# sanweiliti/RoHM

Hardware: AMD Instinct MI355X
Metric: denoised 145-frame clips/sec @1000 DDPM steps (higher is better)
Workload: dtype f32

## Files before the change

rohm_amd/csrc/encoder_chain.hip:

```cpp
#include <type_traits>
#include "common.h"
#include "gemm_sched.h"
#include "attention_tile.h"

namespace rohm {

typedef float f32x16c __attribute__((ext_vector_type(16)));

namespace chain {

constexpr int BM = 144, BK = kGemmBK, NRB = BM / 16;
constexpr int A_UNITS = BM * 8, A_ITERS = (A_UNITS + 255) / 256;
constexpr int kMaxBN = 384;
constexpr int kZone = 2 * (BM + kMaxBN) * BK;
constexpr int kLdsFloats = kZone + 512 + 4 * BM * 2;
constexpr int kSc1 = 16;

struct PhaseArgs {
    const float* A; int lda;
    const float* W; int ldw;
    float* C; int ldc;
    int K;
    const float* bias;
    const float* R; int ldr;
    const float* gamma; const float* beta; float eps; int ln_dim;
    int qcols; float qscale;
    int S; const float* tab; const float* tab0; int ldtab, ldtab0, tab_by_row;
    int m0, n0;
    float* row_stats; unsigned tag28; int tn, tiles_n;
    unsigned* err; unsigned xcc1; int fault;
};

__device__ __forceinline__ int head_row(int n0, int t) { return ((t % 96) >> 5) * 512 + n0 + (t / 96) * 32 + (t & 31); }

template <int BN, bool HEAD = false>
__device__ __forceinline__ void prefetch_w(const float* W, int ldw, int n0, float* smem, int tid, int wave_u) {
    constexpr int B_ITERS = BN * 8 / 256;
    float* Bs = smem + 2 * BM * BK;
#pragma unroll
    for (int buf = 0; buf < 2; ++buf)
#pragma unroll
        for (int i = 0; i < B_ITERS; ++i) {
            const int u = tid + i * 256;
            const int row = u >> 3;
            const int slot = (u & 7) ^ ((row >> 1) & 7);
            const float* src = W + (size_t)(HEAD ? head_row(n0, row) : n0 + row) * ldw + slot * 4 + buf * BK;
            __builtin_amdgcn_global_load_lds((const __attribute__((address_space(1))) void*)src,
                                             (__attribute__((address_space(3))) void*)(Bs + buf * (BN * BK) + (i * 256 + wave_u) * 4), 16, 0, 0);
        }
}

__device__ __forceinline__ void group_sync(unsigned long long* flags, int tn, int G, unsigned tag, unsigned xcc1, unsigned* err, int tid) {
    asm volatile("s_waitcnt vmcnt(0)" ::: "memory");
    __syncthreads();
    if (tid == 0) {
        flags[tn] = ((unsigned long long)xcc1 << 32) | tag;
        asm volatile("" ::: "memory");
    }
    if (tid < G && tid != tn) {
        for (int it = 0;; ++it) {
            const unsigned long long f = __hip_atomic_load(flags + tid, __ATOMIC_RELAXED, __HIP_MEMORY_SCOPE_AGENT);
            if ((unsigned)f == tag && (f >> 32) != 0ull) {
                if ((unsigned)(f >> 32) != xcc1) __hip_atomic_store(err, 2u, __ATOMIC_RELAXED, __HIP_MEMORY_SCOPE_AGENT);
                break;
            }
            __builtin_amdgcn_s_sleep(1);
            if ((it & 127) == 127 && __hip_atomic_load(err, __ATOMIC_RELAXED, __HIP_MEMORY_SCOPE_AGENT) != 0u) break;
            if (it > (1 << 19)) {
                __hip_atomic_store(err, 1u, __ATOMIC_RELAXED, __HIP_MEMORY_SCOPE_AGENT);
                break;
            }
        }
    }
    __syncthreads();
}

template <int BN, int EPI, bool PREF, bool SC1, bool REFETCH, bool HEAD = false, typename AfterLoop>
__device__ __forceinline__ void gemm_phase(const PhaseArgs& p, float* smem, const int tid, AfterLoop&& after_loop,
                                           AtQFrags<2>* q_out = nullptr) {
    static_assert(EPI == EPI_BIAS_RES_LN || EPI == EPI_BIAS_GELU || EPI == EPI_QKV || EPI == EPI_EMBED, "chain phases: LN tail, GELU, QKV, embed");
    static_assert(!HEAD || (EPI == EPI_QKV && BN == 3 * AT_DH), "the head-aligned tile is one head's q | k | v");
    constexpr int WN = BN / 4;
    constexpr int NCB = WN / 16;
    constexpr int B_ITERS = BN * 8 / 256;
    constexpr int PIECES = A_ITERS + B_ITERS;
    constexpr int AUX = SC1 ? kSc1 : 0;

    float* As = smem;
    float* Bs = smem + 2 * BM * BK;
    float* lds_dummy = smem + kZone;
    float* const zone = lds_dummy + 512;
    float* const colrow = HEAD ? smem + 2 * AT_TILE : zone;
    static_assert(!HEAD || 2 * AT_TILE + 512 <= AT_LDS_FLOATS, "head-aligned tile: the bias row overruns the stack's LDS");

    const int lane = tid & 63;
    const int wave = tid >> 6;
    const int li = lane & 15, lg = lane >> 4;
    const int wave_u = __builtin_amdgcn_readfirstlane(wave) * 64;
    const int m0 = p.m0, n0 = p.n0;

    const float* a_src[A_ITERS];
#pragma unroll
    for (int i = 0; i < A_ITERS; ++i) {
        const int u = tid + i * 256;
        const int row = (u < A_UNITS) ? (u >> 3) : 0;
        const int slot = (u & 7) ^ ((row >> 1) & 7);
        a_src[i] = p.A + (size_t)(m0 + row) * p.lda + slot * 4;
    }
    const float* b_src[B_ITERS];
#pragma unroll
    for (int i = 0; i < B_ITERS; ++i) {
        const int u = tid + i * 256;
        const int row = u >> 3;
        const int slot = (u & 7) ^ ((row >> 1) & 7);
        b_src[i] = p.W + (size_t)(HEAD ? head_row(n0, row) : n0 + row) * p.ldw + slot * 4;
    }
    auto dma_a = [&](int buf, int k0) {
#pragma unroll
        for (int piece = 0; piece < A_ITERS; ++piece) {
            float* dst = As + buf * (BM * BK) + (piece * 256 + wave_u) * 4;
            if (piece == A_ITERS - 1 && A_UNITS % 256 != 0)
                dst = (wave_u < A_UNITS - (A_ITERS - 1) * 256) ? dst : lds_dummy + (wave_u & 64) * 4;
            __builtin_amdgcn_global_load_lds((const __attribute__((address_space(1))) void*)(a_src[piece] + k0),
                                             (__attribute__((address_space(3))) void*)dst, 16, 0, AUX);
        }
    };
    auto dma_b = [&](int buf, int k0) {
#pragma unroll
        for (int i = 0; i < B_ITERS; ++i)
            __builtin_amdgcn_global_load_lds((const __attribute__((address_space(1))) void*)(b_src[i] + k0),
                                             (__attribute__((address_space(3))) void*)(Bs + buf * (BN * BK) + (i * 256 + wave_u) * 4), 16, 0, 0);
    };

    f32x4 acc16[NRB * NCB];
#pragma unroll
    for (int i = 0; i < NRB * NCB; ++i) acc16[i] = f32x4{0.f, 0.f, 0.f, 0.f};
    constexpr int READS = NRB + NCB;
    constexpr int MFMAS = 4 * NRB * NCB;
    struct Frag { f32x4 a[NRB]; f32x4 b[NCB]; };
    Frag f0, f1;
    auto read_frags = [&](Frag& f, int buf, int ks) {
        const float* as = As + buf * (BM * BK);
        const float* bs = Bs + buf * (BN * BK) + wave * WN * BK;
        const int slot = ks * 4 + lg;
#pragma unroll
        for (int c = 0; c < NCB; ++c) f.b[c] = *reinterpret_cast<const f32x4*>(bs + lds_off(c * 16 + li, slot));
#pragma unroll
        for (int r = 0; r < NRB; ++r) f.a[r] = *reinterpret_cast<const f32x4*>(as + lds_off(r * 16 + li, slot));
    };
    auto mma_half = [&](const Frag& f) {
#pragma unroll
        for (int r = 0; r < NRB; ++r)
#pragma unroll
            for (int c = 0; c < NCB; ++c)
#pragma unroll
                for (int j = 0; j < 4; ++j)
                    acc16[r * NCB + c] = __builtin_amdgcn_mfma_f32_16x16x4f32(f.b[c][j], f.a[r][j], acc16[r * NCB + c], 0, 0, 0);
    };

    const int nk = p.K / BK;
    constexpr bool COL_LDS = BN >= 384;
    if constexpr (!PREF) { dma_b(0, 0); dma_b(1, BK); }
    if constexpr (COL_LDS) {
        if (wave == 0) {
#pragma unroll
            for (int h = 0; h < 2; ++h) {
                const int unit = h * 64 + lane;
                const int t = (unit < BN / 4 ? unit : BN / 4 - 1) * 4;
                const float* src = HEAD ? p.bias + head_row(n0, t) : p.bias + n0 + t;
                __builtin_amdgcn_global_load_lds((const __attribute__((address_space(1))) void*)src,
                                                 (__attribute__((address_space(3))) void*)(colrow + h * 256), 16, 0, 0);
            }
        }
    }
    dma_a(0, 0);
    dma_a(1, BK);

    const int nw = n0 + wave * WN;
    struct ColOps { f32x4 bias, g4, b4; };
    constexpr bool RES = (EPI == EPI_BIAS_RES_LN);
    constexpr bool HAS_RES = RES || EPI == EPI_EMBED;
    constexpr bool PEEL = BN <= 256;
    constexpr bool EARLY = PEEL && !COL_LDS;
    const f32x4 zero4 = f32x4{0.f, 0.f, 0.f, 0.f};
    auto load_col = [&](int nb) __attribute__((always_inline)) {
        ColOps o{zero4, zero4, zero4};
        if constexpr (EPI == EPI_EMBED) {  }
        else if constexpr (COL_LDS) o.bias = *reinterpret_cast<const f32x4*>(colrow + (nb - n0));
        else o.bias = *reinterpret_cast<const f32x4*>(p.bias + nb);
        if constexpr (RES) {
            o.g4 = *reinterpret_cast<const f32x4*>(p.gamma + nb);
            o.b4 = *reinterpret_cast<const f32x4*>(p.beta + nb);
        }
        return o;
    };
    auto for_units = [&](auto&& fn) __attribute__((always_inline)) {
#pragma unroll
        for (int r = 0; r < NRB; ++r)
#pragma unroll
            for (int c = 0; c < NCB; ++c) fn(c * NRB + r, c, m0 + r * 16 + li, nw + c * 16 + lg * 4, acc16[r * NCB + c]);
    };
    ColOps col[NCB];
    f32x4 res[HAS_RES ? NCB * NRB : 1];
    auto request_ops = [&]() __attribute__((always_inline)) {
#pragma unroll
        for (int c = 0; c < NCB; ++c) col[c] = load_col(nw + c * 16 + lg * 4);
        if constexpr (RES)
            for_units([&](int i, int, int m, int nb, f32x4) __attribute__((always_inline)) {
                res[i] = *reinterpret_cast<const f32x4*>(p.R + (size_t)m * p.ldr + nb);
            });
        if constexpr (EPI == EPI_EMBED)
            for_units([&](int i, int, int m, int nb, f32x4) __attribute__((always_inline)) {
                const int bidx = m / p.S, tok = m % p.S;
                const float* tp = (tok == 0) ? p.tab0 + (size_t)bidx * p.ldtab0 + nb : p.tab + (size_t)(p.tab_by_row ? m : tok) * p.ldtab + nb;
                res[i] = *reinterpret_cast<const f32x4*>(tp);
            });
    };

    asm volatile("s_waitcnt vmcnt(%0)" ::"n"(A_ITERS) : "memory");
    __syncthreads();
    read_frags(f0, 0, 0);
    constexpr int NG = READS;
    constexpr int MF = (MFMAS + NG - 1) / NG;
    auto chunk = [&](int kc, auto last_tag, auto dma_tag) __attribute__((always_inline)) {
        constexpr bool LAST = decltype(last_tag)::value;
        constexpr bool DMA = decltype(dma_tag)::value;
        const int buf = kc & 1;
        if constexpr (LAST && EARLY) request_ops();
        read_frags(f1, buf, 1);
        mma_half(f0);
        SchedGroups<0, NG, MF, READS, 0, 0>::run();
        __builtin_amdgcn_sched_barrier(0);
        if constexpr (!LAST) {
            asm volatile("s_waitcnt vmcnt(0)" ::: "memory");
            __syncthreads();
            __builtin_amdgcn_sched_barrier(0);
            if constexpr (DMA) {
                const int kn = ((kc + 2 < nk) ? (kc + 2) : (nk - 1)) * BK;
                dma_a(buf, kn);
                dma_b(buf, kn);
            }
            read_frags(f0, buf ^ 1, 0);
            mma_half(f1);
            SchedGroups<0, NG, MF, READS, DMA ? PIECES : 0, 1>::run();
        } else {
            mma_half(f1);
        }
        __builtin_amdgcn_sched_barrier(0);
    };
    using DmaTail = std::integral_constant<bool, REFETCH>;
    if constexpr (PEEL) {
        for (int kc = 0; kc + 2 < nk; ++kc) chunk(kc, std::false_type{}, std::true_type{});
        chunk(nk - 2, std::false_type{}, DmaTail{});
        chunk(nk - 1, std::true_type{}, std::false_type{});
    } else {
        for (int kc = 0; kc + 2 < nk; ++kc) chunk(kc, std::false_type{}, std::true_type{});
        chunk(nk - 2, std::false_type{}, DmaTail{});
        chunk(nk - 1, std::false_type{}, DmaTail{});
    }
    asm volatile("s_waitcnt vmcnt(0)" ::: "memory");
    __syncthreads();
    after_loop();
    if constexpr (!EARLY) request_ops();

    if constexpr (EPI == EPI_BIAS_RES_LN) {
#pragma unroll
        for (int c = 0; c < NCB; ++c)
#pragma unroll
            for (int r = 0; r < NRB; ++r) {
                f32x4& a = acc16[r * NCB + c];
                const f32x4 rr = res[c * NRB + r];
#pragma unroll
                for (int q = 0; q < 4; ++q) a[q] = (a[q] + col[c].bias[q]) + rr[q];
            }
        typedef unsigned rohm_u2 __attribute__((ext_vector_type(2)));
        auto merge_swap = [](float& m, float& q2, float n, bool far) __attribute__((always_inline)) {
            rohm_u2 tm, tq;
            if (far) { tm = __builtin_amdgcn_permlane32_swap(__float_as_uint(m), __float_as_uint(m), false, false);
                       tq = __builtin_amdgcn_permlane32_swap(__float_as_uint(q2), __float_as_uint(q2), false, false); }
            else     { tm = __builtin_amdgcn_permlane16_swap(__float_as_uint(m), __float_as_uint(m), false, false);
                       tq = __builtin_amdgcn_permlane16_swap(__float_as_uint(q2), __float_as_uint(q2), false, false); }
            const float ma = __uint_as_float(tm[0]), mb = __uint_as_float(tm[1]);
            const float d = mb - ma;
            m = 0.5f * (ma + mb);
            q2 = (__uint_as_float(tq[0]) + __uint_as_float(tq[1])) + 0.5f * n * d * d;
        };
        float* const part = zone;
        constexpr float kLane = (float)(4 * NCB);
#pragma unroll
        for (int r = 0; r < NRB; ++r) {
            float sm = 0.f;
#pragma unroll
            for (int c = 0; c < NCB; ++c)
#pragma unroll
                for (int k = 0; k < 4; ++k) sm += acc16[r * NCB + c][k];
            float m = sm * (1.0f / kLane), q2 = 0.f;
#pragma unroll
            for (int c = 0; c < NCB; ++c)
#pragma unroll
                for (int k = 0; k < 4; ++k) { const float d = acc16[r * NCB + c][k] - m; q2 += d * d; }
            merge_swap(m, q2, kLane, true);
            merge_swap(m, q2, 2.0f * kLane, false);
            if (lg == 0) *reinterpret_cast<f32x2*>(part + (wave * BM + r * 16 + li) * 2) = f32x2{m, q2};
        }
        __syncthreads();
        const int tn = p.tn, tiles_n = p.tiles_n;
        const unsigned xcc1 = p.xcc1, ep28 = p.tag28;
        const unsigned tag = (ep28 << 4) | xcc1;
        float* const row_stats = p.row_stats;
        if (tid < BM) {
            auto merge = [](float ma, float qa, float mb, float qb, float n, float& m, float& q2) __attribute__((always_inline)) {
                const float d = mb - ma;
                m = 0.5f * (ma + mb);
                q2 = (qa + qb) + 0.5f * n * d * d;
            };
            f32x2 w4[4];
#pragma unroll
            for (int w = 0; w < 4; ++w) w4[w] = *reinterpret_cast<const f32x2*>(part + (w * BM + tid) * 2);
            float m01, q01, m23, q23, a, b;
            merge(w4[0][0], w4[0][1], w4[1][0], w4[1][1], (float)WN, m01, q01);
            merge(w4[2][0], w4[2][1], w4[3][0], w4[3][1], (float)WN, m23, q23);
            merge(m01, q01, m23, q23, 2.0f * (float)WN, a, b);
            const unsigned pub = (p.fault && tn == 0) ? (tag ^ 0x80000000u) : tag;
            *reinterpret_cast<f32x4*>(row_stats + ((size_t)tn * BM + tid) * 4) = f32x4{a, __uint_as_float(pub), b, __uint_as_float(pub)};
            float mk[8], qk[8];
            for (int it = 0;; ++it) {
                unsigned long long lo[8], hi[8];
#pragma unroll
                for (int k = 0; k < 8; ++k) {
                    lo[k] = hi[k] = 0ull;
                    if (k < tiles_n && k != tn) {
                        const unsigned long long* sp = reinterpret_cast<const unsigned long long*>(row_stats + ((size_t)k * BM + tid) * 4);
                        lo[k] = __hip_atomic_load(sp, __ATOMIC_RELAXED, __HIP_MEMORY_SCOPE_AGENT);
                        hi[k] = __hip_atomic_load(sp + 1, __ATOMIC_RELAXED, __HIP_MEMORY_SCOPE_AGENT);
                    }
                }
                bool ok = true, same_xcd = true;
#pragma unroll
                for (int k = 0; k < 8; ++k) {
                    mk[k] = 0.f; qk[k] = 0.f;
                    if (k >= tiles_n) continue;
                    if (k == tn) { mk[k] = a; qk[k] = b; continue; }
                    const unsigned tl = (unsigned)(lo[k] >> 32), th = (unsigned)(hi[k] >> 32);
                    ok = ok && (tl >> 4) == ep28 && (th >> 4) == ep28 && (tl & 15u) != 0u && (th & 15u) != 0u;
                    same_xcd = same_xcd && (tl & 15u) == xcc1 && (th & 15u) == xcc1;
                    mk[k] = __uint_as_float((unsigned)lo[k]);
                    qk[k] = __uint_as_float((unsigned)hi[k]);
                }
                if (ok) {
                    if (!same_xcd) __hip_atomic_store(p.err, 2u, __ATOMIC_RELAXED, __HIP_MEMORY_SCOPE_AGENT);
                    break;
                }
                __builtin_amdgcn_s_sleep(1);
                if ((it & 127) == 127 && __hip_atomic_load(p.err, __ATOMIC_RELAXED, __HIP_MEMORY_SCOPE_AGENT) != 0u) break;
                if (it > (1 << 19)) {
                    __hip_atomic_store(p.err, 1u, __ATOMIC_RELAXED, __HIP_MEMORY_SCOPE_AGENT);
                    break;
                }
            }
            constexpr float kT = (float)BN;
            if (tiles_n > 1) {
                merge(mk[0], qk[0], mk[1], qk[1], kT, mk[0], qk[0]);
                if (tiles_n > 2) merge(mk[2], qk[2], mk[3], qk[3], kT, mk[2], qk[2]);
                if (tiles_n > 4) { merge(mk[4], qk[4], mk[5], qk[5], kT, mk[4], qk[4]); merge(mk[6], qk[6], mk[7], qk[7], kT, mk[6], qk[6]); }
            }
            if (tiles_n > 2) {
                merge(mk[0], qk[0], mk[2], qk[2], 2.0f * kT, mk[0], qk[0]);
                if (tiles_n > 4) merge(mk[4], qk[4], mk[6], qk[6], 2.0f * kT, mk[4], qk[4]);
            }
            if (tiles_n > 4) merge(mk[0], qk[0], mk[4], qk[4], 4.0f * kT, mk[0], qk[0]);
            const float mu = mk[0];
            const float var = qk[0] / (float)p.ln_dim;
            *reinterpret_cast<f32x2*>(part + tid * 2) = f32x2{mu, 1.0f / sqrtf(var + p.eps)};
        }
        __syncthreads();
#pragma unroll
        for (int r = 0; r < NRB; ++r) {
            const f32x2 mrv = *reinterpret_cast<const f32x2*>(part + (r * 16 + li) * 2);
#pragma unroll
            for (int c = 0; c < NCB; ++c) {
                const f32x4 a = acc16[r * NCB + c];
                f32x4 v;
#pragma unroll
                for (int q = 0; q < 4; ++q) v[q] = (a[q] - mrv[0]) * mrv[1] * col[c].g4[q] + col[c].b4[q];
                *reinterpret_cast<f32x4*>(p.C + (size_t)(m0 + r * 16 + li) * p.ldc + nw + c * 16 + lg * 4) = v;
            }
        }
    } else if constexpr (HEAD) {
        float* const Ks = smem;
        float* const Vs = smem + AT_TILE;
        auto put = [&](float* img, int c) __attribute__((always_inline)) {
            const int u = wave * 8 + (c & 1) * 4 + lg;
#pragma unroll
            for (int r = 0; r < NRB; ++r) {
                const f32x4 a = acc16[r * NCB + c];
                f32x4 v;
#pragma unroll
                for (int q = 0; q < 4; ++q) v[q] = a[q] + col[c].bias[q];
                if (c < 2) {
#pragma unroll
                    for (int q = 0; q < 4; ++q) v[q] *= p.qscale;
                }
                *reinterpret_cast<f32x4*>(img + (r * 16 + li) * AT_DH + ((u ^ li) << 2)) = v;
            }
        };
        put(Vs, 0); put(Vs, 1);
        put(Ks, 2); put(Ks, 3);
        __syncthreads();
#pragma unroll
        for (int ks = 0; ks < 8; ++ks) {
            const int sw = ((ks * 4 + lg) ^ li) << 2;
#pragma unroll
            for (int ps = 0; ps < 2; ++ps) q_out->f[ps][ks] = *reinterpret_cast<const f32x4*>(Vs + ((ps * 4 + wave) * 16 + li) * AT_DH + sw);
            q_out->c[ks] = *reinterpret_cast<const f32x4*>(Vs + (8 * 16 + li) * AT_DH + sw);
        }
        __syncthreads();
        put(Vs, 4); put(Vs, 5);
    } else if constexpr (EPI == EPI_EMBED) {
        for_units([&](int i, int, int m, int nb, f32x4 a) __attribute__((always_inline)) {
            const int tok = m % p.S;
            f32x4 v;
#pragma unroll
            for (int q = 0; q < 4; ++q) v[q] = (tok == 0 ? 0.f : a[q]) + res[i][q];
            *reinterpret_cast<f32x4*>(p.C + (size_t)m * p.ldc + nb) = v;
        });
    } else {
        for_units([&](int, int cg, int m, int nb, f32x4 a) __attribute__((always_inline)) {
            f32x4 v;
#pragma unroll
            for (int q = 0; q < 4; ++q) v[q] = a[q] + col[cg].bias[q];
            if constexpr (EPI == EPI_BIAS_GELU) {
#pragma unroll
                for (int q = 0; q < 4; ++q) v[q] = gelu_erf(v[q]);
            }
            if constexpr (EPI == EPI_QKV) {
                if (nb < p.qcols) {
#pragma unroll
                    for (int q = 0; q < 4; ++q) v[q] *= p.qscale;
                }
            }
            *reinterpret_cast<f32x4*>(p.C + (size_t)m * p.ldc + nb) = v;
        });
    }
}

template <int G>
__device__ __forceinline__ void head_tail_phase(const StackParams& p, const int g, const int tn, float* smem, const int tid) {
    constexpr int NC_OWN = 16 / G;
    constexpr int NW = NC_OWN * 16 + 16;
    constexpr int NRMAX = (G == 4) ? 9 : 5;
    constexpr int W_UNITS = NW * 8, W_ITERS = (W_UNITS + 255) / 256;
    constexpr int PIECES = A_ITERS + W_ITERS;
    constexpr int kBuf = (BM + NW) * BK;
    static_assert(3 * kBuf <= kZone, "head phase: staging buffers overrun the zone");
    float* lds_dummy = smem + kZone;
    const int lane = tid & 63, li = lane & 15, lg = lane >> 4;
    const int wave = __builtin_amdgcn_readfirstlane(tid >> 6);
    const int wave_u = wave * 64;
    const int D = p.D, m0 = g * BM;
    int c_loc, r0, nr, e;
    if constexpr (G == 4) { c_loc = wave; r0 = 0; nr = 9; e = tn * 4 + wave; }
    else { c_loc = wave >> 1; r0 = (wave & 1) ? 5 : 0; nr = (wave & 1) ? 4 : 5; e = (wave & 1) ? tn * 2 + (wave >> 1) : 99; }
    const bool has_e = e < NRB;

    const float* a_src[A_ITERS];
#pragma unroll
    for (int i = 0; i < A_ITERS; ++i) {
        const int u = tid + i * 256;
        const int row = (u < A_UNITS) ? (u >> 3) : 0;
        const int slot = (u & 7) ^ ((row >> 1) & 7);
        a_src[i] = p.h + (size_t)(m0 + row) * D + slot * 4;
    }
    const float* w_src[W_ITERS];
#pragma unroll
    for (int i = 0; i < W_ITERS; ++i) {
        const int u = tid + i * 256;
        const int lrow = (u < W_UNITS) ? (u >> 3) : 0;
        const int slot = (u & 7) ^ ((lrow >> 1) & 7);
        const int grow = (lrow < NC_OWN * 16) ? tn * NC_OWN * 16 + lrow : 256 + (lrow - NC_OWN * 16);
        w_src[i] = p.t_out_w + (size_t)grow * D + slot * 4;
    }
    auto dma = [&](int buf, int k0) {
#pragma unroll
        for (int i = 0; i < A_ITERS; ++i) {
            float* dst = smem + buf * kBuf + (i * 256 + wave_u) * 4;
            if (i == A_ITERS - 1 && A_UNITS % 256 != 0)
                dst = (wave_u < A_UNITS - (A_ITERS - 1) * 256) ? dst : lds_dummy + (wave_u & 64) * 4;
            __builtin_amdgcn_global_load_lds((const __attribute__((address_space(1))) void*)(a_src[i] + k0),
                                             (__attribute__((address_space(3))) void*)dst, 16, 0, kSc1);
        }
#pragma unroll
        for (int i = 0; i < W_ITERS; ++i) {
            float* dst = smem + buf * kBuf + BM * BK + (i * 256 + wave_u) * 4;
            if (i == W_ITERS - 1 && W_UNITS % 256 != 0)
                dst = (wave_u < W_UNITS - (W_ITERS - 1) * 256) ? dst : lds_dummy + (wave_u & 64) * 4;
            __builtin_amdgcn_global_load_lds((const __attribute__((address_space(1))) void*)(w_src[i] + k0),
                                             (__attribute__((address_space(3))) void*)dst, 16, 0, 0);
        }
    };

    f32x4 acc[NRMAX], acc_e = f32x4{0.f, 0.f, 0.f, 0.f};
#pragma unroll
    for (int r = 0; r < NRMAX; ++r) acc[r] = f32x4{0.f, 0.f, 0.f, 0.f};
    const int nk = D / BK;
    dma(0, 0);
    dma(1, BK);

    typedef float f32x4u __attribute__((ext_vector_type(4), aligned(4)));
    const int C = p.t_C, T = p.t_T, traj = p.t_traj, S = BM;
    float* const x = p.t_x;
    const float* const nzp = p.t_noise;
    const size_t row_own = ((size_t)g * C + traj + (tn * NC_OWN + c_loc) * 16 + li) * T;
    const size_t row_sh = ((size_t)g * C + traj + 256 + li) * T;
    f32x4 xt[NRMAX], nz[NRMAX], xt_e = f32x4{0.f, 0.f, 0.f, 0.f}, nz_e = f32x4{0.f, 0.f, 0.f, 0.f};
#pragma unroll
    for (int r = 0; r < NRMAX; ++r) {
        xt[r] = nz[r] = f32x4{0.f, 0.f, 0.f, 0.f};
        if (r < nr) {
            const size_t idx = row_own + (size_t)((r0 + r) * 16 + 4 * lg) - 1;
            xt[r] = *reinterpret_cast<const f32x4u*>(x + idx);
            if (nzp) nz[r] = *reinterpret_cast<const f32x4u*>(nzp + idx);
        }
    }
    if (has_e) {
        const size_t idx = row_sh + (size_t)(e * 16 + 4 * lg) - 1;
        xt_e = *reinterpret_cast<const f32x4u*>(x + idx);
        if (nzp) nz_e = *reinterpret_cast<const f32x4u*>(nzp + idx);
    }
    const float bias_own = p.t_out_b[(tn * NC_OWN + c_loc) * 16 + li], bias_sh = p.t_out_b[256 + li];
    struct HFrag { f32x4 a[NRMAX]; f32x4 ae, w, wsh; };
    auto read_h = [&](HFrag& f, int b, int ks) __attribute__((always_inline)) {
        const float* as = smem + b * kBuf;
        const float* ws = as + BM * BK;
        const int slot = ks * 4 + lg;
        f.w = *reinterpret_cast<const f32x4*>(ws + lds_off(c_loc * 16 + li, slot));
#pragma unroll
        for (int r = 0; r < NRMAX; ++r)
            if (r < nr) f.a[r] = *reinterpret_cast<const f32x4*>(as + lds_off((r0 + r) * 16 + li, slot));
        if (has_e) {
            f.ae = *reinterpret_cast<const f32x4*>(as + lds_off(e * 16 + li, slot));
            f.wsh = *reinterpret_cast<const f32x4*>(ws + lds_off(NC_OWN * 16 + li, slot));
        }
    };
    auto mma_h = [&](const HFrag& f) __attribute__((always_inline)) {
#pragma unroll
        for (int r = 0; r < NRMAX; ++r)
            if (r < nr) {
#pragma unroll
                for (int j = 0; j < 4; ++j) acc[r] = __builtin_amdgcn_mfma_f32_16x16x4f32(f.a[r][j], f.w[j], acc[r], 0, 0, 0);
            }
        if (has_e) {
#pragma unroll
            for (int j = 0; j < 4; ++j) acc_e = __builtin_amdgcn_mfma_f32_16x16x4f32(f.ae[j], f.wsh[j], acc_e, 0, 0, 0);
        }
    };
    HFrag f0, f1;
    f0.ae = f0.wsh = f1.ae = f1.wsh = f32x4{0.f, 0.f, 0.f, 0.f};
#pragma unroll
    for (int r = 0; r < NRMAX; ++r) f0.a[r] = f1.a[r] = f32x4{0.f, 0.f, 0.f, 0.f};
    asm volatile("s_waitcnt vmcnt(0)" ::: "memory");
    __syncthreads();
    read_h(f0, 0, 0);
    int buf = 0;
    for (int kc = 0; kc < nk; ++kc) {
        AT_WAIT_LGKM0();
        __builtin_amdgcn_sched_barrier(0);
        read_h(f1, buf, 1);
        __builtin_amdgcn_sched_barrier(0);
        mma_h(f0);
        __builtin_amdgcn_sched_barrier(0);
        const int nbuf = buf == 2 ? 0 : buf + 1;
        if (kc + 1 < nk) {
            asm volatile("s_waitcnt vmcnt(0)" ::: "memory");
            __syncthreads();
            __builtin_amdgcn_sched_barrier(0);
            if (kc + 2 < nk) dma(buf >= 1 ? buf - 1 : 2, (kc + 2) * BK);
            AT_WAIT_LGKM0();
            __builtin_amdgcn_sched_barrier(0);
            read_h(f0, nbuf, 0);
            __builtin_amdgcn_sched_barrier(0);
        } else {
            AT_WAIT_LGKM0();
        }
        mma_h(f1);
        __builtin_amdgcn_sched_barrier(0);
        buf = nbuf;
    }

    const float c1 = p.t_c1, c2 = p.t_c2, sg = p.t_sigma;
    float* const x0o = p.t_x0;
    float* const apk = p.t_apack;
    auto emit = [&](int rblk, size_t row, int ch, float bias, const f32x4& a, const f32x4& xv, const f32x4& nv) __attribute__((always_inline)) {
        const int tok0 = rblk * 16 + 4 * lg;
        f32x4 val, o;
#pragma unroll
        for (int v = 0; v < 4; ++v) {
            val[v] = a[v] + bias;
            o[v] = c1 * val[v] + c2 * xv[v];
            if (nzp) o[v] += sg * nv[v];
        }
        const size_t idx = row + (size_t)tok0 - 1;
        if (tok0 != 0) {
            if (x0o) *reinterpret_cast<f32x4u*>(x0o + idx) = val;
            *reinterpret_cast<f32x4u*>(x + idx) = o;
        } else {
#pragma unroll
            for (int v = 1; v < 4; ++v) {
                if (x0o) x0o[idx + v] = val[v];
                x[idx + v] = o[v];
            }
        }
        if (apk) {
            float* const d = apk + ((size_t)g * S + tok0) * p.t_lda + traj + ch;
#pragma unroll
            for (int v = 0; v < 4; ++v)
                if (tok0 + v != 0) d[(size_t)v * p.t_lda] = o[v];
        }
    };
#pragma unroll
    for (int r = 0; r < NRMAX; ++r)
        if (r < nr) emit(r0 + r, row_own, (tn * NC_OWN + c_loc) * 16 + li, bias_own, acc[r], xt[r], nz[r]);
    if (has_e) emit(e, row_sh, 256 + li, bias_sh, acc_e, xt_e, nz_e);
    for (int i = tn * 256 + tid; i < traj * T; i += G * 256) {
        const int ch = i / T, t = i - ch * T;
        const size_t idx = ((size_t)g * C + ch) * T + t;
        const float val = p.t_cond[idx];
        if (x0o) x0o[idx] = val;
        float o = c1 * val + c2 * x[idx];
        if (nzp) o += sg * nzp[idx];
        x[idx] = o;
        if (apk) apk[((size_t)g * S + t + 1) * p.t_lda + ch] = o;
    }
}

}

template <int G>
__global__ __launch_bounds__(256) void encoder_chain_kernel(ChainParams p) {
    using namespace chain;
    constexpr int BNL = 512 / G, BNF = 1024 / G, BNQ = 1536 / G;
    extern __shared__ __attribute__((aligned(16))) float smem[];
    const int tid = threadIdx.x;
    const int wave_u = __builtin_amdgcn_readfirstlane(tid >> 6) * 64;
    const int x = blockIdx.x % kNumXCD, j = blockIdx.x / kNumXCD;
    const int g = (j / G) * kNumXCD + x, tn = j % G;
    if (g >= p.tiles_m) return;
    const unsigned xcc1 = 1u + (unsigned)__builtin_amdgcn_s_getreg((3 << 11) | 20);
    const unsigned ep = p.epoch + 64u * *p.xln_pass;
    if (tid == 0) p.xln_xcc[g * 8 + tn] = xcc1;
    unsigned long long* const flags = p.flags + (size_t)g * 9 * 5 * 8;

    PhaseArgs a{};
    a.m0 = g * BM; a.err = p.xln_err; a.xcc1 = xcc1; a.tn = tn; a.tiles_n = G;
    a.row_stats = p.xln_stats + ((size_t)g * G * BM) * 4;
    a.eps = p.ln_eps; a.ln_dim = p.D;

    a.A = p.ctx; a.lda = p.D; a.W = p.out_w; a.ldw = p.D; a.C = p.y; a.ldc = p.D; a.K = p.D; a.bias = p.out_b;
    a.R = p.h; a.ldr = p.D; a.gamma = p.n1_w; a.beta = p.n1_b; a.n0 = tn * BNL; a.tag28 = ep & 0x0fffffffu; a.fault = p.fault & 1;
    gemm_phase<BNL, EPI_BIAS_RES_LN, false, false, G == 8>(a, smem, tid, [&]() { prefetch_w<BNF>(p.l1_w, p.D, tn * BNF, smem, tid, wave_u); });
    group_sync(flags, tn, G, ep, xcc1, p.xln_err, tid);

    a.A = p.y; a.lda = p.D; a.W = p.l1_w; a.ldw = p.D; a.C = p.ff; a.ldc = p.F; a.K = p.D; a.bias = p.l1_b; a.n0 = tn * BNF;
    gemm_phase<BNF, EPI_BIAS_GELU, true, true, G == 8>(a, smem, tid, [&]() { prefetch_w<BNL>(p.l2_w, p.F, tn * BNL, smem, tid, wave_u); });
    group_sync(flags + 8, tn, G, ep, xcc1, p.xln_err, tid);

    a.A = p.ff; a.lda = p.F; a.W = p.l2_w; a.ldw = p.F; a.C = p.h; a.ldc = p.D; a.K = p.F; a.bias = p.l2_b;
    a.R = p.y; a.ldr = p.D; a.gamma = p.n2_w; a.beta = p.n2_b; a.n0 = tn * BNL; a.tag28 = (ep + 1u) & 0x0fffffffu; a.fault = (p.fault >> 1) & 1;
    gemm_phase<BNL, EPI_BIAS_RES_LN, true, true, G == 8>(a, smem, tid, [&]() { if (p.qkv) prefetch_w<BNQ>(p.in_w, p.D, tn * BNQ, smem, tid, wave_u); });
    if (p.qkv == nullptr) return;
    group_sync(flags + 16, tn, G, ep, xcc1, p.xln_err, tid);

    a.A = p.h; a.lda = p.D; a.W = p.in_w; a.ldw = p.D; a.C = p.qkv; a.ldc = 3 * p.D; a.K = p.D; a.bias = p.in_b; a.n0 = tn * BNQ;
    a.qcols = p.D; a.qscale = p.qscale;
    gemm_phase<BNQ, EPI_QKV, true, true, G == 8>(a, smem, tid, []() {});
}

template <int G>
__global__ __launch_bounds__(256) void encoder_stack_kernel(StackParams p) {
    using namespace chain;
    constexpr int BNL = 512 / G, BNF = 1024 / G, BNQ = 1536 / G;
    extern __shared__ __attribute__((aligned(16))) float smem[];
    const int tid0 = threadIdx.x;
    const int x = blockIdx.x % kNumXCD, j = blockIdx.x / kNumXCD;
    const int g = (j / G) * kNumXCD + x, tn = j % G;
    if (g >= p.tiles_m) return;
    const unsigned xcc1 = 1u + (unsigned)__builtin_amdgcn_s_getreg((3 << 11) | 20);
    const unsigned ep = p.epoch + 64u * (*p.xln_pass + p.pass_add);
    if (tid0 == 0) p.xln_xcc[g * 8 + tn] = xcc1;

    PhaseArgs a{};
    a.m0 = g * BM; a.err = p.xln_err; a.xcc1 = xcc1; a.tn = tn; a.tiles_n = G;
    a.row_stats = p.xln_stats + ((size_t)g * G * BM) * 4;
    a.eps = p.ln_eps; a.ln_dim = p.D;
    a.qcols = p.D; a.qscale = p.qscale;
    constexpr bool HEAD = G == 4;
    auto n0q = [&]() __attribute__((always_inline)) { return HEAD ? tn * AT_DH : tn * BNQ; };
    AtQFrags<2> qh;
    unsigned long long* const tl = p.timeline ? p.timeline + (size_t)blockIdx.x * kStackTimelineLayers * kStackTimelineStamps : nullptr;
    auto stamp = [&](int layer, int k) __attribute__((always_inline)) {
        if (tl != nullptr && threadIdx.x == 0) tl[layer * kStackTimelineStamps + k] = __builtin_amdgcn_s_memrealtime();
    };
    auto attend = [&](int l, int tid) __attribute__((always_inline)) {
        unsigned long long* const fl = p.flags + ((size_t)g * 9 + l) * 5 * 8;
        stamp(l, 0);
        if (l > 0) {
            if constexpr (HEAD) __syncthreads();
            else group_sync(fl, tn, G, ep, xcc1, p.xln_err, tid);
        }
        stamp(l, 1);
        if constexpr (HEAD)
            attention_item<4, 0, kSc1, 2, true>(p.qkv, p.ctx, p.n_head, g * p.n_head + tn, 0, AT_NB, smem, tid, &qh);
        else attention_item<4, 0, kSc1, 1>(p.qkv, p.ctx, p.n_head, g * p.n_head + (tn >> 1), (tn & 1) ? 5 : 0, (tn & 1) ? 4 : 5, smem, tid);
        stamp(l, 2);
        group_sync(fl + 8, tn, G, ep, xcc1, p.xln_err, tid);
        stamp(l, 3);
    };
    {
    int tid = tid0;
    asm volatile("" : "+v"(tid));
    const int wave_u = __builtin_amdgcn_readfirstlane(tid >> 6) * 64;
    unsigned long long* const fl = p.flags + ((size_t)g * 9 + 8) * 5 * 8;
    a.A = p.apack; a.lda = p.lda_pack; a.W = p.w_embed; a.ldw = p.ldw_embed; a.C = p.h; a.ldc = p.D; a.K = p.k_embed; a.n0 = tn * BNL;
    a.S = p.S; a.tab = p.tab; a.tab0 = p.tab0; a.ldtab = p.ldtab; a.ldtab0 = p.ldtab0; a.tab_by_row = p.tab_by_row;
    stamp(8, 0);
    gemm_phase<BNL, EPI_EMBED, false, false, G == 8>(a, smem, tid, [&]() { prefetch_w<BNQ, HEAD>(p.layer[0].in_w, p.D, n0q(), smem, tid, wave_u); });
    stamp(8, 1);
    group_sync(fl, tn, G, ep, xcc1, p.xln_err, tid);
    stamp(8, 2);
    a.A = p.h; a.lda = p.D; a.W = p.layer[0].in_w; a.ldw = p.D; a.C = p.qkv; a.ldc = 3 * p.D; a.K = p.D; a.bias = p.layer[0].in_b;
    a.n0 = n0q();
    gemm_phase<BNQ, EPI_QKV, true, true, G == 8, HEAD>(a, smem, tid, []() {}, &qh);
    stamp(8, 3);
    if constexpr (HEAD) __syncthreads();
    else group_sync(fl + 8, tn, G, ep, xcc1, p.xln_err, tid);
    stamp(8, 4);
    if constexpr (HEAD) attend(0, tid);
    }
#pragma unroll 1
    for (int l = 0; l < p.L; ++l) {
        int tid = tid0;
        asm volatile("" : "+v"(tid));
        const int wave_u = __builtin_amdgcn_readfirstlane(tid >> 6) * 64;
        const StackLayerW& w = p.layer[l];
        unsigned long long* const fl = p.flags + ((size_t)g * 9 + l) * 5 * 8;
        if constexpr (!HEAD) attend(l, tid);

        a.A = p.ctx; a.lda = p.D; a.W = w.out_w; a.ldw = p.D; a.C = p.y; a.ldc = p.D; a.K = p.D; a.bias = w.out_b;
        a.R = p.h; a.ldr = p.D; a.gamma = w.n1_w; a.beta = w.n1_b; a.n0 = tn * BNL; a.tag28 = (ep + 4u * l) & 0x0fffffffu;
        a.fault = (l == 0) ? (p.fault & 1) : 0;
        gemm_phase<BNL, EPI_BIAS_RES_LN, false, true, G == 8>(a, smem, tid, [&]() { prefetch_w<BNF>(w.l1_w, p.D, tn * BNF, smem, tid, wave_u); });
        stamp(l, 4);
        group_sync(fl + 16, tn, G, ep, xcc1, p.xln_err, tid);
        stamp(l, 5);

        a.A = p.y; a.lda = p.D; a.W = w.l1_w; a.ldw = p.D; a.C = p.ff; a.ldc = p.F; a.K = p.D; a.bias = w.l1_b; a.n0 = tn * BNF;
        gemm_phase<BNF, EPI_BIAS_GELU, true, true, G == 8>(a, smem, tid, [&]() { prefetch_w<BNL>(w.l2_w, p.F, tn * BNL, smem, tid, wave_u); });
        stamp(l, 6);
        group_sync(fl + 24, tn, G, ep, xcc1, p.xln_err, tid);
        stamp(l, 7);

        const bool more = l + 1 < p.L;
        a.A = p.ff; a.lda = p.F; a.W = w.l2_w; a.ldw = p.F; a.C = p.h; a.ldc = p.D; a.K = p.F; a.bias = w.l2_b;
        a.R = p.y; a.ldr = p.D; a.gamma = w.n2_w; a.beta = w.n2_b; a.n0 = tn * BNL; a.tag28 = (ep + 4u * l + 1u) & 0x0fffffffu;
        a.fault = (l == 0) ? ((p.fault >> 1) & 1) : 0;
        gemm_phase<BNL, EPI_BIAS_RES_LN, true, true, G == 8>(a, smem, tid, [&]() { if (more) prefetch_w<BNQ, HEAD>(p.layer[l + 1].in_w, p.D, n0q(), smem, tid, wave_u); });
        stamp(l, 8);
        if (!more) {
            if (p.tail) {
                group_sync(fl + 32, tn, G, ep, xcc1, p.xln_err, tid);
                stamp(l, 9);
                head_tail_phase<G>(p, g, tn, smem, tid);
                stamp(l, 10);
                if (p.t_pass_ctr != nullptr && blockIdx.x == 0 && threadIdx.x == 0) p.t_pass_ctr[1] = p.pass_add + 1u;
            }
            break;
        }
        group_sync(fl + 32, tn, G, ep, xcc1, p.xln_err, tid);
        stamp(l, 9);

        a.A = p.h; a.lda = p.D; a.W = p.layer[l + 1].in_w; a.ldw = p.D; a.C = p.qkv; a.ldc = 3 * p.D; a.K = p.D; a.bias = p.layer[l + 1].in_b;
        a.n0 = n0q();
        gemm_phase<BNQ, EPI_QKV, true, true, G == 8, HEAD>(a, smem, tid, []() {}, &qh);
        stamp(l, 10);
        if constexpr (HEAD) attend(l + 1, tid);
    }
}

int launch_encoder_stack(const StackParams& p, hipStream_t s) {
    const int G = encoder_chain_parts(p.M, p.D, p.F);
    ROHM_ARG_CHECK(G != 0 && p.n_head == 4 && p.L >= 1 && p.L <= 8, "encoder_stack: shape (M %d, D %d, F %d, %d heads, %d layers) has no stack form",
                   p.M, p.D, p.F, p.n_head, p.L);
    ROHM_ARG_CHECK(p.h && p.y && p.ff && p.qkv && p.ctx && p.xln_stats && p.xln_err && p.xln_pass && p.xln_xcc && p.flags, "encoder_stack: null operand");
    ROHM_ARG_CHECK(p.apack && p.w_embed && p.tab && p.tab0 && p.S == chain::BM && p.k_embed >= 2 * chain::BK && p.k_embed % chain::BK == 0 &&
                       p.lda_pack % 4 == 0 && p.ldw_embed % 4 == 0 && p.ldtab % 4 == 0 && p.ldtab0 % 4 == 0,
                   "encoder_stack: bad operands of the leading embed phase");
    StackParams q = p;
    q.tiles_m = p.M / chain::BM;
    const int groups8 = (q.tiles_m + kNumXCD - 1) / kNumXCD * kNumXCD;
    ROHM_ARG_CHECK(!p.tail || (p.D == 512 && p.t_out_w && p.t_out_b && p.t_x && p.t_cond && p.t_C - p.t_traj == 272 &&
                               p.t_T == chain::BM - 1 && p.t_traj > 0 && (!p.t_apack || p.t_lda >= p.t_C)),
                   "encoder_stack: the closing head / update / pack phase needs whole 144-token clips, d_model 512 and 272 predicted channels");
    constexpr int kFloats = AT_LDS_FLOATS > chain::kLdsFloats ? AT_LDS_FLOATS : chain::kLdsFloats;
    const size_t lds = (size_t)kFloats * sizeof(float);
    static bool attr_set[64][2] = {};
    int dev = 0;
    ROHM_HIP_CHECK(hipGetDevice(&dev));
    if (dev < 64 && !attr_set[dev][G == 8]) {
        if (G == 4) ROHM_HIP_CHECK(hipFuncSetAttribute(reinterpret_cast<const void*>(&encoder_stack_kernel<4>), hipFuncAttributeMaxDynamicSharedMemorySize, (int)lds));
        else ROHM_HIP_CHECK(hipFuncSetAttribute(reinterpret_cast<const void*>(&encoder_stack_kernel<8>), hipFuncAttributeMaxDynamicSharedMemorySize, (int)lds));
        attr_set[dev][G == 8] = true;
    }
    const double MM = (double)p.M, D = p.D, F = p.F, L = p.L;
    const double flops = L * (4.0 * 144.0 * 128.0 * MM * p.n_head + 2.0 * MM * (D * D + 2.0 * D * F)) + L * 2.0 * MM * 3.0 * D * D +
                         2.0 * MM * D * p.k_embed;
    const double bytes = 4.0 * (L * (MM * (3.0 * D + D + 4.0 * D + 2.0 * F + D) + D * D + 2.0 * D * F) + (L - 1.0) * (MM * 3.0 * D + 3.0 * D * D));
    const double tail_flops = p.tail ? 2.0 * MM * D * (p.t_C - p.t_traj) : 0.0;
    prof::Scope ps(p.tail ? "gemm_stack_tail" : "gemm_stack", flops + tail_flops, bytes, s);
    if (G == 4) hipLaunchKernelGGL(encoder_stack_kernel<4>, dim3(groups8 * 4), dim3(256), lds, s, q);
    else hipLaunchKernelGGL(encoder_stack_kernel<8>, dim3(groups8 * 8), dim3(256), lds, s, q);
    ROHM_LAUNCH_CHECK();
    return ROHM_OK;
}

int encoder_chain_parts(int M, int D, int F) {
    if (D != 512 || F != 1024 || M <= 0 || M % chain::BM != 0) return 0;
    const int tm = M / chain::BM;
    return tm >= 48 ? 4 : 8;
}

bool encoder_chain_pays(int B) {
    if (B <= 0) return false;
    if (B < 48) return B > 24 && B <= 32;
    if (B <= 64) return true;
    const int wgs = (B + kNumXCD - 1) / kNumXCD * kNumXCD * 4, rounds = (wgs + 255) / 256;
    return 4 * B * 100 >= 93 * rounds * 256;
}

size_t encoder_chain_flag_bytes(int M) { return (size_t)((M + chain::BM - 1) / chain::BM) * 9 * 5 * 8 * sizeof(unsigned long long); }

int launch_encoder_chain(const ChainParams& p, hipStream_t s) {
    const int G = encoder_chain_parts(p.M, p.D, p.F);
    ROHM_ARG_CHECK(G != 0, "encoder_chain: shape (M %d, D %d, F %d) has no chain form", p.M, p.D, p.F);
    ROHM_ARG_CHECK(p.ctx && p.h && p.y && p.ff && p.out_w && p.out_b && p.n1_w && p.n1_b && p.l1_w && p.l1_b && p.l2_w && p.l2_b &&
                       p.n2_w && p.n2_b && p.xln_stats && p.xln_err && p.xln_pass && p.xln_xcc && p.flags && (!p.qkv || (p.in_w && p.in_b)),
                   "encoder_chain: null operand");
    ChainParams q = p;
    q.tiles_m = p.M / chain::BM;
    const int groups8 = (q.tiles_m + kNumXCD - 1) / kNumXCD * kNumXCD;
    const size_t lds = (size_t)chain::kLdsFloats * sizeof(float);
    static bool attr_set[64][2] = {};
    int dev = 0;
    ROHM_HIP_CHECK(hipGetDevice(&dev));
    if (dev < 64 && !attr_set[dev][G == 8]) {
        if (G == 4) ROHM_HIP_CHECK(hipFuncSetAttribute(reinterpret_cast<const void*>(&encoder_chain_kernel<4>), hipFuncAttributeMaxDynamicSharedMemorySize, (int)lds));
        else ROHM_HIP_CHECK(hipFuncSetAttribute(reinterpret_cast<const void*>(&encoder_chain_kernel<8>), hipFuncAttributeMaxDynamicSharedMemorySize, (int)lds));
        attr_set[dev][G == 8] = true;
    }
    const double MM = (double)p.M, D = p.D, F = p.F;
    const double flops = 2.0 * MM * (D * D + 2.0 * D * F + (p.qkv ? 3.0 * D * D : 0.0));
    const double bytes = 4.0 * (MM * (4.0 * D + 2.0 * F + D + (p.qkv ? 3.0 * D : 0.0)) + D * D + 2.0 * D * F + (p.qkv ? 3.0 * D * D : 0.0));
    prof::Scope ps(p.qkv ? "gemm_chain" : "gemm_chain_last", flops, bytes, s);
    if (G == 4) hipLaunchKernelGGL(encoder_chain_kernel<4>, dim3(groups8 * 4), dim3(256), lds, s, q);
    else hipLaunchKernelGGL(encoder_chain_kernel<8>, dim3(groups8 * 8), dim3(256), lds, s, q);
    ROHM_LAUNCH_CHECK();
    return ROHM_OK;
}

}
```

Before: 23.50.

## Replace group barriers with deferred polling using per-tile rotated K order

In the 4-way head-aligned mode, each block now starts its next GEMM at a K offset rotated by its tile index, so it first consumes its own producer's columns. The group barrier becomes a publish-only flag write. The wait on the other blocks' flags is folded into the K loop at the chunk just before foreign data is needed. This lets blocks overlap useful work with the inter-block sync instead of stalling at a full barrier. It adds complexity, and correctness depends on the rotation matching which A columns each peer produced.

```diff
diff --git a/rohm_amd/csrc/encoder_chain.hip b/rohm_amd/csrc/encoder_chain.hip
--- a/rohm_amd/csrc/encoder_chain.hip
+++ b/rohm_amd/csrc/encoder_chain.hip
@@ -29,12 +29,13 @@
     int m0, n0;
     float* row_stats; unsigned tag28; int tn, tiles_n;
     unsigned* err; unsigned xcc1; int fault;
+    const unsigned long long* poll; unsigned poll_tag;
 };
 
 __device__ __forceinline__ int head_row(int n0, int t) { return ((t % 96) >> 5) * 512 + n0 + (t / 96) * 32 + (t & 31); }
 
 template <int BN, bool HEAD = false>
-__device__ __forceinline__ void prefetch_w(const float* W, int ldw, int n0, float* smem, int tid, int wave_u) {
+__device__ __forceinline__ void prefetch_w(const float* W, int ldw, int n0, float* smem, int tid, int wave_u, int krot = 0) {
     constexpr int B_ITERS = BN * 8 / 256;
     float* Bs = smem + 2 * BM * BK;
 #pragma unroll
@@ -44,7 +45,7 @@
             const int u = tid + i * 256;
             const int row = u >> 3;
             const int slot = (u & 7) ^ ((row >> 1) & 7);
-            const float* src = W + (size_t)(HEAD ? head_row(n0, row) : n0 + row) * ldw + slot * 4 + buf * BK;
+            const float* src = W + (size_t)(HEAD ? head_row(n0, row) : n0 + row) * ldw + slot * 4 + buf * BK + krot;
             __builtin_amdgcn_global_load_lds((const __attribute__((address_space(1))) void*)src,
                                              (__attribute__((address_space(3))) void*)(Bs + buf * (BN * BK) + (i * 256 + wave_u) * 4), 16, 0, 0);
         }
@@ -75,7 +76,31 @@
     __syncthreads();
 }
 
-template <int BN, int EPI, bool PREF, bool SC1, bool REFETCH, bool HEAD = false, typename AfterLoop>
+__device__ __forceinline__ void group_publish(unsigned long long* flags, int tn, unsigned tag, unsigned xcc1, int tid) {
+    asm volatile("s_waitcnt vmcnt(0)" ::: "memory");
+    __syncthreads();
+    if (tid == 0) {
+        flags[tn] = ((unsigned long long)xcc1 << 32) | tag;
+        asm volatile("" ::: "memory");
+    }
+}
+__device__ __forceinline__ void group_poll_rest(const unsigned long long* flag, unsigned long long f, unsigned tag, unsigned xcc1, unsigned* err) {
+    for (int it = 0;; ++it) {
+        if ((unsigned)f == tag && (f >> 32) != 0ull) {
+            if ((unsigned)(f >> 32) != xcc1) __hip_atomic_store(err, 2u, __ATOMIC_RELAXED, __HIP_MEMORY_SCOPE_AGENT);
+            break;
+        }
+        __builtin_amdgcn_s_sleep(1);
+        if ((it & 127) == 127 && __hip_atomic_load(err, __ATOMIC_RELAXED, __HIP_MEMORY_SCOPE_AGENT) != 0u) break;
+        if (it > (1 << 19)) {
+            __hip_atomic_store(err, 1u, __ATOMIC_RELAXED, __HIP_MEMORY_SCOPE_AGENT);
+            break;
+        }
+        f = __hip_atomic_load(flag, __ATOMIC_RELAXED, __HIP_MEMORY_SCOPE_AGENT);
+    }
+}
+
+template <int BN, int EPI, bool PREF, bool SC1, bool REFETCH, bool HEAD = false, bool ROT = false, typename AfterLoop>
 __device__ __forceinline__ void gemm_phase(const PhaseArgs& p, float* smem, const int tid, AfterLoop&& after_loop,
                                            AtQFrags<2>* q_out = nullptr) {
     static_assert(EPI == EPI_BIAS_RES_LN || EPI == EPI_BIAS_GELU || EPI == EPI_QKV || EPI == EPI_EMBED, "chain phases: LN tail, GELU, QKV, embed");
@@ -160,7 +185,9 @@
 
     const int nk = p.K / BK;
     constexpr bool COL_LDS = BN >= 384;
-    if constexpr (!PREF) { dma_b(0, 0); dma_b(1, BK); }
+    const int rot = ROT ? p.tn * (nk >> 2) : 0;
+    auto kmap = [&](int kc) __attribute__((always_inline)) { return ROT ? ((kc + rot) & (nk - 1)) * BK : kc * BK; };
+    if constexpr (!PREF) { dma_b(0, kmap(0)); dma_b(1, kmap(1)); }
     if constexpr (COL_LDS) {
         if (wave == 0) {
 #pragma unroll
@@ -173,8 +200,8 @@
             }
         }
     }
-    dma_a(0, 0);
-    dma_a(1, BK);
+    dma_a(0, kmap(0));
+    dma_a(1, kmap(1));
 
     const int nw = n0 + wave * WN;
     struct ColOps { f32x4 bias, g4, b4; };
@@ -222,6 +249,7 @@
     read_frags(f0, 0, 0);
     constexpr int NG = READS;
     constexpr int MF = (MFMAS + NG - 1) / NG;
+    const int poll_kc = (nk >> 2) - 2;
     auto chunk = [&](int kc, auto last_tag, auto dma_tag) __attribute__((always_inline)) {
         constexpr bool LAST = decltype(last_tag)::value;
         constexpr bool DMA = decltype(dma_tag)::value;
@@ -232,11 +260,23 @@
         SchedGroups<0, NG, MF, READS, 0, 0>::run();
         __builtin_amdgcn_sched_barrier(0);
         if constexpr (!LAST) {
-            asm volatile("s_waitcnt vmcnt(0)" ::: "memory");
+            if constexpr (ROT && DMA) {
+                if (kc == poll_kc) {
+                    const bool poller = tid < 4 && tid != p.tn;
+                    unsigned long long f = 0ull;
+                    if (poller) f = __hip_atomic_load(p.poll + tid, __ATOMIC_RELAXED, __HIP_MEMORY_SCOPE_AGENT);
+                    asm volatile("s_waitcnt vmcnt(0)" ::: "memory");
+                    if (poller) group_poll_rest(p.poll + tid, f, p.poll_tag, p.xcc1, p.err);
+                } else {
+                    asm volatile("s_waitcnt vmcnt(0)" ::: "memory");
+                }
+            } else {
+                asm volatile("s_waitcnt vmcnt(0)" ::: "memory");
+            }
             __syncthreads();
             __builtin_amdgcn_sched_barrier(0);
             if constexpr (DMA) {
-                const int kn = ((kc + 2 < nk) ? (kc + 2) : (nk - 1)) * BK;
+                const int kn = kmap((kc + 2 < nk) ? (kc + 2) : (nk - 1));
                 dma_a(buf, kn);
                 dma_b(buf, kn);
             }
@@ -696,6 +736,12 @@
     constexpr bool HEAD = G == 4;
     auto n0q = [&]() __attribute__((always_inline)) { return HEAD ? tn * AT_DH : tn * BNQ; };
     AtQFrags<2> qh;
+    constexpr bool ROT = HEAD;
+    auto meet = [&](unsigned long long* f, int tid) __attribute__((always_inline)) {
+        if constexpr (ROT) { group_publish(f, tn, ep, xcc1, tid); a.poll = f; a.poll_tag = ep; }
+        else group_sync(f, tn, G, ep, xcc1, p.xln_err, tid);
+    };
+    auto krot = [&](int K) __attribute__((always_inline)) { return ROT ? tn * (K >> 2) : 0; };
     unsigned long long* const tl = p.timeline ? p.timeline + (size_t)blockIdx.x * kStackTimelineLayers * kStackTimelineStamps : nullptr;
     auto stamp = [&](int layer, int k) __attribute__((always_inline)) {
         if (tl != nullptr && threadIdx.x == 0) tl[layer * kStackTimelineStamps + k] = __builtin_amdgcn_s_memrealtime();
@@ -712,7 +758,7 @@
             attention_item<4, 0, kSc1, 2, true>(p.qkv, p.ctx, p.n_head, g * p.n_head + tn, 0, AT_NB, smem, tid, &qh);
         else attention_item<4, 0, kSc1, 1>(p.qkv, p.ctx, p.n_head, g * p.n_head + (tn >> 1), (tn & 1) ? 5 : 0, (tn & 1) ? 4 : 5, smem, tid);
         stamp(l, 2);
-        group_sync(fl + 8, tn, G, ep, xcc1, p.xln_err, tid);
+        meet(fl + 8, tid);
         stamp(l, 3);
     };
     {
@@ -723,13 +769,13 @@
     a.A = p.apack; a.lda = p.lda_pack; a.W = p.w_embed; a.ldw = p.ldw_embed; a.C = p.h; a.ldc = p.D; a.K = p.k_embed; a.n0 = tn * BNL;
     a.S = p.S; a.tab = p.tab; a.tab0 = p.tab0; a.ldtab = p.ldtab; a.ldtab0 = p.ldtab0; a.tab_by_row = p.tab_by_row;
     stamp(8, 0);
-    gemm_phase<BNL, EPI_EMBED, false, false, G == 8>(a, smem, tid, [&]() { prefetch_w<BNQ, HEAD>(p.layer[0].in_w, p.D, n0q(), smem, tid, wave_u); });
+    gemm_phase<BNL, EPI_EMBED, false, false, G == 8>(a, smem, tid, [&]() { prefetch_w<BNQ, HEAD>(p.layer[0].in_w, p.D, n0q(), smem, tid, wave_u, krot(p.D)); });
     stamp(8, 1);
-    group_sync(fl, tn, G, ep, xcc1, p.xln_err, tid);
+    meet(fl, tid);
     stamp(8, 2);
     a.A = p.h; a.lda = p.D; a.W = p.layer[0].in_w; a.ldw = p.D; a.C = p.qkv; a.ldc = 3 * p.D; a.K = p.D; a.bias = p.layer[0].in_b;
     a.n0 = n0q();
-    gemm_phase<BNQ, EPI_QKV, true, true, G == 8, HEAD>(a, smem, tid, []() {}, &qh);
+    gemm_phase<BNQ, EPI_QKV, true, true, G == 8, HEAD, ROT>(a, smem, tid, []() {}, &qh);
     stamp(8, 3);
     if constexpr (HEAD) __syncthreads();
     else group_sync(fl + 8, tn, G, ep, xcc1, p.xln_err, tid);
@@ -748,22 +794,23 @@
         a.A = p.ctx; a.lda = p.D; a.W = w.out_w; a.ldw = p.D; a.C = p.y; a.ldc = p.D; a.K = p.D; a.bias = w.out_b;
         a.R = p.h; a.ldr = p.D; a.gamma = w.n1_w; a.beta = w.n1_b; a.n0 = tn * BNL; a.tag28 = (ep + 4u * l) & 0x0fffffffu;
         a.fault = (l == 0) ? (p.fault & 1) : 0;
-        gemm_phase<BNL, EPI_BIAS_RES_LN, false, true, G == 8>(a, smem, tid, [&]() { prefetch_w<BNF>(w.l1_w, p.D, tn * BNF, smem, tid, wave_u); });
+        gemm_phase<BNL, EPI_BIAS_RES_LN, false, true, G == 8, false, ROT>(a, smem, tid, [&]() { prefetch_w<BNF>(w.l1_w, p.D, tn * BNF, smem, tid, wave_u, krot(p.D)); });
         stamp(l, 4);
-        group_sync(fl + 16, tn, G, ep, xcc1, p.xln_err, tid);
+        meet(fl + 16, tid);
         stamp(l, 5);
 
         a.A = p.y; a.lda = p.D; a.W = w.l1_w; a.ldw = p.D; a.C = p.ff; a.ldc = p.F; a.K = p.D; a.bias = w.l1_b; a.n0 = tn * BNF;
-        gemm_phase<BNF, EPI_BIAS_GELU, true, true, G == 8>(a, smem, tid, [&]() { prefetch_w<BNL>(w.l2_w, p.F, tn * BNL, smem, tid, wave_u); });
+        gemm_phase<BNF, EPI_BIAS_GELU, true, true, G == 8, false, ROT>(a, smem, tid, [&]() { prefetch_w<BNL>(w.l2_w, p.F, tn * BNL, smem, tid, wave_u, krot(p.F)); });
         stamp(l, 6);
-        group_sync(fl + 24, tn, G, ep, xcc1, p.xln_err, tid);
+        meet(fl + 24, tid);
         stamp(l, 7);
 
         const bool more = l + 1 < p.L;
+        if constexpr (ROT) asm volatile("" : "+v"(tid));
         a.A = p.ff; a.lda = p.F; a.W = w.l2_w; a.ldw = p.F; a.C = p.h; a.ldc = p.D; a.K = p.F; a.bias = w.l2_b;
         a.R = p.y; a.ldr = p.D; a.gamma = w.n2_w; a.beta = w.n2_b; a.n0 = tn * BNL; a.tag28 = (ep + 4u * l + 1u) & 0x0fffffffu;
         a.fault = (l == 0) ? ((p.fault >> 1) & 1) : 0;
-        gemm_phase<BNL, EPI_BIAS_RES_LN, true, true, G == 8>(a, smem, tid, [&]() { if (more) prefetch_w<BNQ, HEAD>(p.layer[l + 1].in_w, p.D, n0q(), smem, tid, wave_u); });
+        gemm_phase<BNL, EPI_BIAS_RES_LN, true, true, G == 8, false, ROT>(a, smem, tid, [&]() { if (more) prefetch_w<BNQ, HEAD>(p.layer[l + 1].in_w, p.D, n0q(), smem, tid, wave_u, krot(p.D)); });
         stamp(l, 8);
         if (!more) {
             if (p.tail) {
@@ -775,12 +822,12 @@
             }
             break;
         }
-        group_sync(fl + 32, tn, G, ep, xcc1, p.xln_err, tid);
+        meet(fl + 32, tid);
         stamp(l, 9);
 
         a.A = p.h; a.lda = p.D; a.W = p.layer[l + 1].in_w; a.ldw = p.D; a.C = p.qkv; a.ldc = 3 * p.D; a.K = p.D; a.bias = p.layer[l + 1].in_b;
         a.n0 = n0q();
-        gemm_phase<BNQ, EPI_QKV, true, true, G == 8, HEAD>(a, smem, tid, []() {}, &qh);
+        gemm_phase<BNQ, EPI_QKV, true, true, G == 8, HEAD, ROT>(a, smem, tid, []() {}, &qh);
         stamp(l, 10);
         if constexpr (HEAD) attend(l + 1, tid);
     }
```

After: 23.24. 1.1% lower.
